# dhansmair/flamingo-mini

Measured on AMD Instinct MI355X. Metric: images/sec (fwd+bwd) flamingo-mini bs=32, higher is better.
Workload: dtype bf16

## Files before the change

### flamingo-mini_amd/csrc/ff_api.hip

```cpp
#include <stdarg.h>
#include <stdio.h>
#include <math.h>
#include <stdlib.h>
#include "ff_common.h"
#include "ff_internal.h"

namespace ff {

static thread_local char g_err[512] = "";
void set_error(const char* fmt, ...) {
    va_list ap;
    va_start(ap, fmt);
    vsnprintf(g_err, sizeof(g_err), fmt, ap);
    va_end(ap);
}
#ifdef FF_DEBUG
int dbg_switch(const char* name, int dflt) {
    const char* e = getenv(name);
    return e ? atoi(e) : dflt;
}
#endif
int check_launch(const char* what) {
    hipError_t e = hipGetLastError();
    if (e != hipSuccess) {
// ... 76 lines not shown
    }
    o.x_last = a.take(rows_q * s.D * s.es);
    o.mean_o = a.take<float>(rows_q * 4);
    o.rstd_o = a.take<float>(rows_q * 4);
    return align_up(a.used);
}

static size_t rs_ws_bytes(const RsDims& s) {
    size_t w = 0;
    auto g = [&](int M, int N, int K, int nz) { w = std::max(w, gemm_workspace_bytes(s.dt, M, N, K, nz, 0)); };
    g(s.Mq, s.inner, s.D, 1); g(s.Mkv, s.inner, s.D, 2); g(s.Mq, s.D, s.inner, 1); g(s.Mq, s.ffi, s.D, 1); g(s.Mq, s.D, s.ffi, 1);
    for (int nz = 1; nz <= 4; nz++) {
        g(s.D, s.ffi, s.Mq, nz); g(s.ffi, s.D, s.Mq, nz); g(s.D, s.inner, s.Mq, nz); g(s.inner, s.D, s.Mq, nz); g(s.inner, s.D, s.Mkv, nz);
    }
    g(s.Mkv, s.D, s.inner, 1);
    w = std::max(w, layernorm_bwd_workspace(s.Mf, s.D));
    w = std::max(w, layernorm_bwd_workspace(s.Mq, s.D));
    w = std::max(w, rows_reduce_workspace(s.Mq, s.D, s.q, 1));
    w = std::max(w, rows_reduce_workspace(s.Mf, s.D, s.F, s.v));
    return align_up(w) + align_up(s.attn_ws);
}
struct RsChain {
    void *ws, *dxn, *dO, *dkv, *dln;
    size_t ws_bytes, gws;
    float* attn_ws;
};
struct RsLayerGrads {
    void *dx_mid, *dH, *dQs, *dK, *dV;
};
static void rs_take_ws(const RsDims& s, Arena& a, RsChain& c) {
// ... 98 lines not shown
    if (partial)
        return layernorm_bwd(a, dy, x, add, gamma, mean, rstd, dx, dx_res, dg, db, partial, layernorm_bwd_partial_bytes(a.rows, a.cols), st, nullptr, pending);
    return layernorm_bwd(a, dy, x, add, gamma, mean, rstd, dx, dx_res, dg, db, W.ws, W.gws, st);
}

static int rs_layer_backward(const RsDims& s, const void* const* p, void* const* g, const void* x_f, const void* tpe, const float* mean_m,
                             const float* rstd_m, const void* x_in, RowMap x_map, const RsLayerSaved& L, const void* dx_out, void* dx_in,
                             void* dx_f, const void* dx_f_res, const RsChain& W, const RsLayerGrads& T, float* const* lnp, LnPending* ln_sets,
                             hipStream_t st) {
    const RowMap pD = s.pD, pI = s.pI, pF = s.pF;
    FF_TRY(Gemm(s.dt, s.Mq, s.ffi, s.D).a(0, pD).b(1, pF).c(pF).act_bwd(s.act).problem(dx_out, p[11], T.dH, nullptr, L.Hpre).run(W.ws, W.gws, st));
    FF_TRY(Gemm(s.dt, s.Mq, s.D, s.ffi).a(0, pF).b(1, pD).c(pD).problem(T.dH, p[10], W.dxn).run(W.ws, W.gws, st));
    FF_TRY(rs_ln_bwd(W, lnp[0], &ln_sets[0], s.ln_latents(), W.dxn, L.x_mid, nullptr, p[8], L.mean_f, L.rstd_f, T.dx_mid, dx_out, g[8], g[9], st));
    FF_TRY(Gemm(s.dt, s.Mq, s.inner, s.D).a(0, pD).b(1, pI).c(pI).problem(T.dx_mid, p[7], W.dO).run(W.ws, W.gws, st));
    FF_TRY(attention_bwd(rs_attn_desc(s), L.Qs, L.K, L.V, nullptr, L.O, W.dO, L.lse, T.dQs, T.dK, T.dV, W.attn_ws, s.attn_ws, st));
    FF_TRY(Gemm(s.dt, s.Mkv, s.D, s.inner).a(0, pI).b(1, pD).c(pD).problem(T.dK, p[5], W.dkv).run(W.ws, W.gws, st));
    FF_TRY(Gemm(s.dt, s.Mkv, s.D, s.inner).a(0, pI).b(1, pD).c(pD).problem(T.dV, p[6], W.dkv, nullptr, nullptr, W.dkv).run(W.ws, W.gws, st));
    FF_TRY(Gemm(s.dt, s.Mq, s.D, s.inner).a(0, pI).b(1, pD).c(pD).res_map(s.kv_lat).scale(s.scale)
               .problem(T.dQs, p[4], W.dln, nullptr, nullptr, s.kv_latent_rows(W.dkv)).run(W.ws, W.gws, st));
    FF_TRY(rs_ln_bwd(W, lnp[1], &ln_sets[1], ln_args(s.dt, s.Mq, s.D, x_map, pD, pD), W.dln, x_in, nullptr, p[2], L.mean_l, L.rstd_l, dx_in, T.dx_mid, g[2],
                     g[3], st));
    return rs_ln_bwd(W, lnp[2], &ln_sets[2], s.ln_media(s.kv_media), W.dkv, x_f, tpe, p[0], mean_m, rstd_m, dx_f, dx_f_res, g[0], g[1], st);
}

static int rs_input_grads(const RsDims& s, const void* dx0, const void* dxf, void* d_latents, void* d_tpe, void* ws, size_t ws_bytes, hipStream_t st) {
    FF_TRY(rows_reduce(s.dt, s.Mq, s.D, s.pD, s.q, 1, dx0, d_latents, ws, ws_bytes, st));
    if (s.nte > s.T) FF_TRY(zero_bytes((char*)d_tpe + (size_t)s.T * s.D * s.es, (size_t)(s.nte - s.T) * s.D * s.es, st));
    return rows_reduce(s.dt, s.Mf, s.D, s.pD, s.F, s.v, dxf, d_tpe, ws, ws_bytes, st);
}

static int resampler_fwd(const ff_resampler_desc* d, const void* x_f, const void* const* P, void* out, void* saved, size_t saved_bytes,
                         void* scratch, size_t scratch_bytes, hipStream_t st) {
// ... 517 lines not shown
    }
    if (finish_ln) FF_TRY(layernorm_bwd_finish(s.dt, ln_sets, 2 * n, st));
    FF_TRY(g3.run(ws, ws_bytes, st));
    FF_TRY(g1.run(ws, ws_bytes, st));
    FF_TRY(go.run(ws, ws_bytes, st));
    return gq.run(ws, ws_bytes, st);
}

static int kvp_check(const ff_kvproj_desc* d) {
    FF_CHECK(d, FF_ERR_SHAPE, "kv_project: null descriptor");
    FF_CHECK(d->dtype == FF_DTYPE_F32 || d->dtype == FF_DTYPE_BF16, FF_ERR_UNSUPPORTED, "kv_project: dtype %d", d->dtype);
    FF_CHECK(d->n_layers > 0 && d->rows > 0 && d->dim_visual > 0 && d->kv_dim > 0 && (long long)d->rows * d->dim_visual < (1LL << 31), FF_ERR_SHAPE,
             "kv_project: bad dimensions");
    return FF_OK;
}
static size_t kvp_gemm_ws(const ff_kvproj_desc* d) {
    size_t w = 0;
    for (int z = 1; z <= kKvProjGroup; z++)
        w = std::max({w, gemm_workspace_bytes(d->dtype, d->rows, d->kv_dim, d->dim_visual, z, 0),
                      gemm_workspace_bytes(d->dtype, d->kv_dim, d->dim_visual, d->rows, z, 0),
                      gemm_workspace_bytes(d->dtype, d->rows, d->dim_visual, d->kv_dim, z, 0)});
    return align_up(w);
}
static size_t kvp_ws_bytes(const ff_kvproj_desc* d, bool with_dvf) {
    const size_t es = d->dtype == FF_DTYPE_BF16 ? 2 : 4;
    size_t w = kvp_gemm_ws(d);
    if (with_dvf)
        w += align_up((size_t)d->n_layers * d->rows * d->dim_visual * es) +
             align_up(rows_reduce_workspace(d->n_layers, d->rows * d->dim_visual, d->n_layers, d->n_layers));
    return w;
}
static int kv_project_fwd(const ff_kvproj_desc* d, const void* vf, const void* const* w_kv, void* const* kv_out, void* ws, size_t ws_bytes,
                          hipStream_t st) {
    FF_TRY(kvp_check(d));
    FF_CHECK(vf && w_kv && kv_out && ws && ws_bytes >= kvp_gemm_ws(d), FF_ERR_WORKSPACE, "kv_project_fwd: null argument or workspace too small");
    const RowMap pV = plain_rows(d->dim_visual), pKV = plain_rows(d->kv_dim);
    for (int l0 = 0; l0 < d->n_layers; l0 += kKvProjGroup) {
        Gemm g(d->dtype, d->rows, d->kv_dim, d->dim_visual);
        g.a(0, pV).b(0, pV).c(pKV);
        for (int l = l0; l < std::min(d->n_layers, l0 + kKvProjGroup); l++) g.problem(vf, w_kv[l], kv_out[l]);
        FF_TRY(g.run(ws, ws_bytes, st));
    }
    return FF_OK;
}
static int kv_project_bwd(const ff_kvproj_desc* d, const void* vf, const void* const* w_kv, const void* const* dkv, void* const* dw_kv,
                          void* dvf, void* ws, size_t ws_bytes, hipStream_t st) {
    FF_TRY(kvp_check(d));
    FF_CHECK(vf && w_kv && dkv && dw_kv && ws && ws_bytes >= kvp_ws_bytes(d, dvf != nullptr), FF_ERR_WORKSPACE,
             "kv_project_bwd: null argument or workspace too small");
    const size_t es = d->dtype == FF_DTYPE_BF16 ? 2 : 4, gws = kvp_gemm_ws(d);
    const RowMap pV = plain_rows(d->dim_visual), pKV = plain_rows(d->kv_dim);
    char* terms = (char*)ws + gws;
    const size_t term_bytes = (size_t)d->rows * d->dim_visual * es;
    for (int l0 = 0; l0 < d->n_layers; l0 += kKvProjGroup) {
        const int l1 = std::min(d->n_layers, l0 + kKvProjGroup);
        Gemm gw(d->dtype, d->kv_dim, d->dim_visual, d->rows);
        gw.a(1, pKV).b(1, pV).c(pV);
        for (int l = l0; l < l1; l++) gw.problem(dkv[l], vf, dw_kv[l]);
        FF_TRY(gw.run(ws, gws, st));
        if (dvf) {
            Gemm gx(d->dtype, d->rows, d->dim_visual, d->kv_dim);
            gx.a(0, pKV).b(1, pV).c(pV);
            for (int l = l0; l < l1; l++) gx.problem(dkv[l], w_kv[l], terms + (size_t)l * term_bytes);
            FF_TRY(gx.run(ws, gws, st));
        }
    }
    if (dvf) {
        const int cols = d->rows * d->dim_visual;
        FF_TRY(rows_reduce(d->dtype, d->n_layers, cols, plain_rows(cols), d->n_layers, d->n_layers, terms, dvf,
                           terms + align_up((size_t)d->n_layers * term_bytes), rows_reduce_workspace(d->n_layers, cols, d->n_layers, d->n_layers), st));
    }
    return FF_OK;
}

}

extern "C" int ff_version(void) { return 6; }
extern "C" const char* ff_arch(void) { return "gfx950"; }
extern "C" const char* ff_last_error(void) { return ff::g_err; }

extern "C" size_t ff_resampler_saved_bytes(const ff_resampler_desc* d) {
    if (ff::rs_check(d) != FF_OK) return 0;
    ff::RsSaved S;
    return ff::rs_saved_layout(ff::RsDims(*d), nullptr, 0, S);
}
// ... 146 lines not shown
```

### flamingo-mini_amd/csrc/ff_gemm.hip

```cpp
#include <atomic>
#include <type_traits>
#include "ff_common.h"
#include <stdlib.h>
#include "ff_internal.h"
#include "ff_gemm_tiles.h"

namespace ff {

template <typename T>
FF_DEV void epilogue4(const GemmParams& P, const GemmProblem& pr, int m, int n, float (&v)[4]) {
    typedef __attribute__((ext_vector_type(4))) T vec4;
    const long long off = P.c_map.off(m) + n;
    const bool full = (n + 3 < P.N);
#pragma unroll
    for (int r = 0; r < 4; r++) v[r] *= P.scale;
    auto load4 = [&](const void* base, long long at, float (&o)[4]) {
        const T* p = (const T*)base + at;
        if (full) {
            vec4 t = *(const vec4*)p;
#pragma unroll
            for (int r = 0; r < 4; r++) o[r] = to_f32(t[r]);
        } else {
#pragma unroll
            for (int r = 0; r < 4; r++) o[r] = (n + r < P.N) ? to_f32(p[r]) : 0.f;
// ... 328 lines not shown
        } else dma_tile_fast<BN, BL, NW>(r, st, v, soff, w);
    }
    static FF_DEV void slow(__amdgpu_buffer_rsrc_t r, bf16* st, const RowMap& map, int n_base, int n_lim, int k0, int k_end, int w, int l, bf16* dummy = nullptr) {
        if constexpr (SPLIT) {
            dma_tile<128, BL, NW>(r, st, map, n_base, n_lim, k0, k_end, w, l);
            if (NW == 8 && w >= 4) dma_tile<32, BL, 4>(r, dummy, map, n_base + 128, 0, k0, k_end, 0, l);
            else dma_tile<32, BL, 4>(r, st + 128 * kBK, map, n_base + 128, n_lim, k0, k_end, w & 3, l);
        } else dma_tile<BN, BL, NW>(r, st, map, n_base, n_lim, k0, k_end, w, l);
    }
    static FF_DEV bf16x8 frag(const bf16* s, int col0, int ks) {
        if constexpr (SPLIT && BL == 1) return col0 < 128 ? frag_read2<128, 1>(s, col0, ks) : frag_read2<32, 1>(s + 128 * kBK, col0 - 128, ks);
        else return frag_read2<BN, BL>(s, col0, ks);
    }
};

template <int BM, int BN, int AL, int BL, int NS, int WPC, int NPW = 4, int NCW = 4>
__global__ __launch_bounds__((NCW + NPW) * 64, WPC * (NCW + NPW) / 4) void gemm_bf16_pc_kernel(const void* hA, const void* hB, int hM, int hN, int hK, int h_split, int h_kps,
                                                           int h_nz, int h_xcd, int h_ald, int h_bld, int h_seg, const GemmParams P) {
    extern __shared__ __attribute__((aligned(16))) unsigned char smem_raw[];
    bf16* smem = (bf16*)smem_raw;
    constexpr int A_ELEMS = BM * kBK, B_ELEMS = BN * kBK, STAGE = A_ELEMS + B_ELEMS;
    constexpr int CM = NCW / 2;
    constexpr int WM = BM / CM, WN = BN / 2, MT = WM / 16, NT = WN / 16;
    static_assert((NCW == 4 || NCW == 8) && WM % 16 == 0, "consumer layout");
    typedef BStage<BN, BL, NPW> BS;
    constexpr int PER_TILE = BM / (NPW * 8) + BS::PER_WAVE;
    static_assert(WN % 16 == 0 && BM % 32 == 0 && BN % 32 == 0, "tile shape");
    static_assert((AL == 0 || BM == 256 || BM == 128 || BM == 64) && (BL == 0 || BN == 128 || BN == 64 || BN == 160), "M-major staging exists for 64 / 128 / 256-wide A tiles and 64 / 128 / 160-wide B tiles only");
    static_assert(PER_TILE * (NS - 1) <= 63, "vmcnt overflow");

    RowMap a_map{h_ald, 0, 0}, b_map{h_bld, 0, 0};
    if (h_seg) { a_map = P.a_map; b_map = P.b_map; }
    const void* opA = hA;
    const void* opB = hB;
    const int tiles_m = (hM + BM - 1) / BM, tiles_n = (hN + BN - 1) / BN;
    const TileCoord tc = tile_coord(h_nz, h_split, h_xcd & 255, h_xcd >> 8, tiles_m, tiles_n);
    if (tc.z > 0) { opA = P.p[tc.z].A; opB = P.p[tc.z].B; }
    const int m_base = tc.tm * BM, n_base = tc.tn * BN;
    const int k_begin = tc.split * h_kps;
    const int k_end = min(hK, k_begin + h_kps);
    const int t = threadIdx.x, l = t & 63;
    const int w = __builtin_amdgcn_readfirstlane(t >> 6);
    const bool producer = w >= NCW;
    const int pw = producer ? w - NCW : w;
    const int wm = (w & (NCW - 1)) >> 1, wn = w & 1;
    bf16* dummy = smem + NS * STAGE + (pw & 3) * 512;
    const __amdgpu_buffer_rsrc_t ra = __builtin_amdgcn_make_buffer_rsrc((void*)opA, 0, 0x7fffffff, 0x00020000);
    const __amdgpu_buffer_rsrc_t rb = __builtin_amdgcn_make_buffer_rsrc((void*)opB, 0, 0x7fffffff, 0x00020000);
    const int nk = (k_end - k_begin + kBK - 1) / kBK;

    f32x4 acc[MT][NT];
#pragma unroll
    for (int i = 0; i < MT; i++)
#pragma unroll
        for (int j = 0; j < NT; j++) acc[i][j] = f32x4{0.f, 0.f, 0.f, 0.f};

    unsigned va[BM / (NPW * 8)], vb[BS::PER_WAVE];
    const bool a_plain = AL == 0 || a_map.rows_per_seg <= 0, b_plain = BL == 0 || b_map.rows_per_seg <= 0;
    const unsigned a_step = AL == 0 ? 2u : (unsigned)a_map.ld * 2u, b_step = BL == 0 ? 2u : (unsigned)b_map.ld * 2u;
    auto issue = [&](int tile) {
        bf16* st = smem + (tile % NS) * STAGE;
        const int k0 = k_begin + tile * kBK;
        const bool full = k0 + kBK <= k_end;
        if (full && a_plain) dma_tile_fast<BM, AL, NPW>(ra, st, va, (unsigned)k0 * a_step, pw);
        else dma_tile<BM, AL, NPW>(ra, st, a_map, m_base, hM, k0, k_end, pw, l);
        if (full && b_plain) BS::fast(rb, st + A_ELEMS, vb, (unsigned)k0 * b_step, pw, dummy);
        else BS::slow(rb, st + A_ELEMS, b_map, n_base, hN, k0, k_end, pw, l, dummy);
    };
    if (producer) {
        dma_prepare<BM, AL, NPW>(a_map, m_base, hM, pw, l, va);
        BS::prepare(b_map, n_base, hN, pw, l, vb);
#pragma unroll
        for (int s = 0; s < NS - 1; s++)
            if (s < nk) issue(s);
    }
    FF_GEMM_ARGS(Q, pr, P);
    if (tc.z > 0) pr = P.p[tc.z];
#ifdef FF_GEMM_PCMODE
    constexpr int pcmode = FF_GEMM_PCMODE;
#else
    constexpr int pcmode = 0;
#endif
    if (producer) {
        for (int kt = 0; kt < nk; kt++) {
            if (pcmode == 2) { __builtin_amdgcn_s_barrier(); continue; }
            const int younger = min(nk - 1 - kt, NS - 2);
            if (NS >= 4 && younger == 2) wait_vmcnt<2 * PER_TILE>();
            else if (NS >= 3 && younger >= 1) wait_vmcnt<PER_TILE>();
            else wait_vmcnt<0>();
            __builtin_amdgcn_s_barrier();
            if (kt + NS - 1 < nk) issue(kt + NS - 1);
        }
// ... 317 lines not shown
#pragma unroll
        for (int j = 0; j < 4; j++) s[(k + j) * kFLd + row] = reg[j];
    } else {
        const int k = t >> 4, row = (t & 15) * 4;
        *(f32x4*)(s + k * kFLd + row) = f32x4{reg[0], reg[1], reg[2], reg[3]};
    }
}

template <int AL, int BL> __global__ __launch_bounds__(256) void gemm_f32_kernel(const GemmParams P) {
    __shared__ __attribute__((aligned(16))) float sA[kFBK * kFLd];
    __shared__ __attribute__((aligned(16))) float sB[kFBK * kFLd];
    const int tiles_m = (P.M + kFBM - 1) / kFBM, tiles_n = (P.N + kFBM - 1) / kFBM;
    const TileCoord tc = tile_coord(P.nz, P.split_k, P.xcd_ms, P.xcd_ns, tiles_m, tiles_n);
    const GemmProblem& pr = P.p[tc.z];
    const int m_base = tc.tm * kFBM, n_base = tc.tn * kFBM;
    const int k_begin = tc.split * P.k_per_split;
    const int k_end = min(P.K, k_begin + P.k_per_split);
    const float* A = (const float*)pr.A;
    const float* B = (const float*)pr.B;
    const int t = threadIdx.x, w = t >> 6, l = t & 63, c = l & 15, g = l >> 4;
    const int wm = w >> 1, wn = w & 1;
    const bool a_vec = P.a_vec_ok, b_vec = P.b_vec_ok;

    f32x4 acc[2][2];
#pragma unroll
    for (int i = 0; i < 2; i++)
#pragma unroll
        for (int j = 0; j < 2; j++) acc[i][j] = f32x4{0.f, 0.f, 0.f, 0.f};

    for (int k0 = k_begin; k0 < k_end; k0 += kFBK) {
        float ra[4], rb[4];
        f32_tile_load<AL>(A, P.a_map, m_base, P.M, k0, k_end, a_vec, ra);
        f32_tile_load<BL>(B, P.b_map, n_base, P.N, k0, k_end, b_vec, rb);
        __syncthreads();
        f32_tile_store<AL>(sA, ra);
        f32_tile_store<BL>(sB, rb);
        __syncthreads();
#pragma unroll
        for (int ks = 0; ks < kFBK / 4; ks++) {
            float fa[2], fb[2];
#pragma unroll
            for (int i = 0; i < 2; i++) fa[i] = sA[(ks * 4 + g) * kFLd + wm * 32 + i * 16 + c];
#pragma unroll
            for (int j = 0; j < 2; j++) fb[j] = sB[(ks * 4 + g) * kFLd + wn * 32 + j * 16 + c];
#pragma unroll
// ... 92 lines not shown
}
int profile_begin(int dtype, int tile, int a_layout, int b_layout, int M, int N, int K, int nz, int split_k, hipStream_t st) {
    if (!g_prof.on.load(std::memory_order_relaxed)) return -1;
    const int i = g_prof.n.fetch_add(1);
    if (i >= g_prof.cap) return -1;
    ff_gemm_profile_record& r = g_prof.rec[i];
    r.dtype = dtype; r.tile = tile; r.a_layout = a_layout; r.b_layout = b_layout;
    r.M = M; r.N = N; r.K = K; r.nz = nz; r.split_k = split_k; r.ms = 0.f;
    hipEventRecord(g_prof.ev[2 * i], st);
    return i;
}
void profile_end(int i, hipStream_t st) {
    if (i >= 0) hipEventRecord(g_prof.ev[2 * i + 1], st);
}
static int prof_begin(const GemmParams& P, int dtype, int bm, hipStream_t st) {
    return profile_begin(dtype, bm, P.a_layout, P.b_layout, P.M, P.N, P.K, P.nz, P.split_k, st);
}
static void prof_end(int i, hipStream_t st) { profile_end(i, st); }

static int env_int(const char* name, int dflt) { return dbg_switch(name, dflt); }

struct TilePlan { int tile, split; };
static TilePlan plan_bf16(int M, int N, int K, int nz, int want_split, int a_layout = 0, int b_layout = 0, int ft = 0) {
    const long long t128 = (long long)cdiv(M, 128) * cdiv(N, 128) * nz, t64 = (long long)cdiv(M, 64) * cdiv(N, 64) * nz;
    TilePlan p;
    static const int env_tile = env_int("FF_GEMM_TILE", 0);
    if (ft == 0) ft = env_tile;
    static const int pc_bl1 = env_int("FF_GEMM_PC_BL1", 1);
    const bool pc_ok = a_layout == 0 && (b_layout == 0 || (pc_bl1 && N % 8 == 0));
    const bool skinny_ok = a_layout == 0 && b_layout == 0;
    const bool rows_ok = skinny_ok && M <= 32 && nz == 1 && K % 32 == 0;
// ... 43 lines not shown
    } else if (t64 >= 200) p = TilePlan{64, 1};
    else {
        int s = (int)std::min<long long>(4, cdiv(256, t64));
        while (s > 1 && K / (64 * s) < 4) s--;
        p = TilePlan{64, s};
    }
    if (want_split > 0) p.split = want_split;
    static const int pc128 = env_int("FF_GEMM_PC128", 2);
    if (pc128 && p.tile == 128) p.tile = 128002;
    if (pc128 >= 2 && p.tile == 6412) p.tile = 128002;
    static const int pc64 = env_int("FF_GEMM_PC64", 1);
    if (pc64 && p.tile == 64) p.tile = 64002;
    return p;
}

template <int BM, int BN, int AL, int BL, int NS> static int launch_bf16_dma(const GemmParams& P, hipStream_t st) {
    constexpr size_t lds = (size_t)NS * (BM + BN) * kBK * sizeof(bf16);
    if (lds > 64 * 1024) {
        static bool attr_done[64] = {};
        int dev = 0;
        (void)hipGetDevice(&dev);
        if (dev < 0 || dev >= 64 || !attr_done[dev]) {
            hipError_t e = hipFuncSetAttribute((const void*)gemm_bf16_dma_kernel<BM, BN, AL, BL, NS>,
                                               hipFuncAttributeMaxDynamicSharedMemorySize, (int)lds);
            FF_CHECK(e == hipSuccess, FF_ERR_LAUNCH, "hipFuncSetAttribute(gemm dma lds=%zu): %s", lds, hipGetErrorString(e));
            if (dev >= 0 && dev < 64) attr_done[dev] = true;
        }
    }
    const int grid = cdiv(P.M, BM) * cdiv(P.N, BN) * P.split_k * P.nz;
    const int seg = P.a_map.rows_per_seg > 0 || P.b_map.rows_per_seg > 0 || P.a_map.ld >= (1LL << 31) || P.b_map.ld >= (1LL << 31);
    gemm_bf16_dma_kernel<BM, BN, AL, BL, NS><<<dim3(grid), dim3(256), lds, st>>>(P.p[0].A, P.p[0].B, P.M, P.N, P.K, P.split_k, P.k_per_split, P.nz,
                                                                           P.xcd_ms | (P.xcd_ns << 8), (int)P.a_map.ld, (int)P.b_map.ld, seg, P);
    return check_launch("gemm_bf16_dma");
}
template <int BM, int BN, int NS> static int dispatch_bf16_dma(const GemmParams& P, hipStream_t st) {
    if (P.a_layout == 0 && P.b_layout == 0) return launch_bf16_dma<BM, BN, 0, 0, NS>(P, st);
    if (P.a_layout == 0 && P.b_layout == 1) return launch_bf16_dma<BM, BN, 0, 1, NS>(P, st);
    if (P.a_layout == 1 && P.b_layout == 0) return launch_bf16_dma<BM, BN, 1, 0, NS>(P, st);
    return launch_bf16_dma<BM, BN, 1, 1, NS>(P, st);
}
template <int BM, int BN> static int run_bf16_dma_tile(const GemmParams& P, int ns, hipStream_t st) {
    return ns == 2 ? dispatch_bf16_dma<BM, BN, 2>(P, st) : ns == 4 ? dispatch_bf16_dma<BM, BN, 4>(P, st) : dispatch_bf16_dma<BM, BN, 3>(P, st);
}
template <int BM, int BN, int AL, int BL, int NS, int WPC, int NPW = 4, int NCW = 4> static int launch_bf16_pc(const GemmParams& P, hipStream_t st) {
    constexpr size_t lds = (size_t)NS * (BM + BN) * kBK * sizeof(bf16) + (NPW == 8 && BN == 160 ? 4096 : 0);
    static bool attr_done[64] = {};
    int dev = 0;
    (void)hipGetDevice(&dev);
    if (dev < 0 || dev >= 64 || !attr_done[dev]) {
        hipError_t e = hipFuncSetAttribute((const void*)gemm_bf16_pc_kernel<BM, BN, AL, BL, NS, WPC, NPW, NCW>, hipFuncAttributeMaxDynamicSharedMemorySize, (int)lds);
        FF_CHECK(e == hipSuccess, FF_ERR_LAUNCH, "hipFuncSetAttribute(gemm pc lds=%zu): %s", lds, hipGetErrorString(e));
        if (dev >= 0 && dev < 64) attr_done[dev] = true;
    }
    const int grid = cdiv(P.M, BM) * cdiv(P.N, BN) * P.split_k * P.nz;
    const int seg = P.a_map.rows_per_seg > 0 || P.b_map.rows_per_seg > 0 || P.a_map.ld >= (1LL << 31) || P.b_map.ld >= (1LL << 31);
    gemm_bf16_pc_kernel<BM, BN, AL, BL, NS, WPC, NPW, NCW><<<dim3(grid), dim3((NCW + NPW) * 64), lds, st>>>(P.p[0].A, P.p[0].B, P.M, P.N, P.K, P.split_k, P.k_per_split,
                                                                                 P.nz, P.xcd_ms | (P.xcd_ns << 8), (int)P.a_map.ld,
                                                                                 (int)P.b_map.ld, seg, P);
    return check_launch("gemm_bf16_pc");
}
template <int NS> static int dispatch_bf16_pc128(const GemmParams& P, hipStream_t st) {
    if (P.a_layout == 0 && P.b_layout == 0) return launch_bf16_pc<128, 128, 0, 0, NS, 2>(P, st);
    if (P.a_layout == 0 && P.b_layout == 1) return launch_bf16_pc<128, 128, 0, 1, NS, 2>(P, st);
    if (P.a_layout == 1 && P.b_layout == 0) return launch_bf16_pc<128, 128, 1, 0, NS, 2>(P, st);
    return launch_bf16_pc<128, 128, 1, 1, NS, 2>(P, st);
}
static int run_bf16_dma(const GemmParams& P, hipStream_t st) {
    static const int ns_env = env_int("FF_GEMM_STAGES", 0);
    const int ns = P.force_stages > 0 ? P.force_stages : ns_env > 0 ? ns_env : 2;
    if (P.tile == 128160) {
        static const int npw_full = env_int("FF_GEMM_NPW", 8), npw_split = env_int("FF_GEMM_NPW_SPLIT", 4);
        const int npw = P.split_k > 1 ? npw_split : npw_full;
        const int pns = P.force_stages > 0 ? P.force_stages : ns_env > 0 ? ns_env : npw == 8 ? 4 : 3;
        static const int ncw_env = env_int("FF_GEMM_NCW", 4), ncw_split_env = env_int("FF_GEMM_NCW_SPLIT", 4);
        const int ncw = P.force_tile == 128168 ? 8 : (P.split_k > 1 ? ncw_split_env : ncw_env);
        if (ncw == 8) {
            if (P.b_layout == 0) return pns == 3 ? launch_bf16_pc<128, 160, 0, 0, 3, 1, 4, 8>(P, st) : launch_bf16_pc<128, 160, 0, 0, 4, 1, 4, 8>(P, st);
            return pns == 3 ? launch_bf16_pc<128, 160, 0, 1, 3, 1, 4, 8>(P, st) : launch_bf16_pc<128, 160, 0, 1, 4, 1, 4, 8>(P, st);
        }
        if (npw == 8) {
            if (P.b_layout == 0) return pns == 4 ? launch_bf16_pc<128, 160, 0, 0, 4, 1, 8>(P, st) : launch_bf16_pc<128, 160, 0, 0, 3, 1, 8>(P, st);
            return pns == 4 ? launch_bf16_pc<128, 160, 0, 1, 4, 1, 8>(P, st) : launch_bf16_pc<128, 160, 0, 1, 3, 1, 8>(P, st);
        }
        if (P.b_layout == 0) return pns == 4 ? launch_bf16_pc<128, 160, 0, 0, 4, 1>(P, st) : launch_bf16_pc<128, 160, 0, 0, 3, 1>(P, st);
// ... 29 lines not shown
    int s = (int)(256 / tiles);
    s = std::min(s, K / 512);
    s = std::min(s, 16);
    return std::max(s, 1);
}

size_t gemm_workspace_bytes(int dtype, int M, int N, int K, int nz, int split_k) {
    if (split_k <= 0) split_k = gemm_pick_split(dtype, M, N, K, nz);
    return split_k > 1 ? (size_t)split_k * nz * M * N * sizeof(float) : 0;
}

int gemm_launch(GemmParams P, int dtype, void* workspace, size_t ws_bytes, hipStream_t st, int* leave_partial) {
    if (leave_partial) *leave_partial = 1;
    FF_CHECK(P.M > 0 && P.N > 0 && P.K > 0 && P.nz >= 1 && P.nz <= kGemmMaxZ, FF_ERR_SHAPE, "gemm: bad shape M=%d N=%d K=%d nz=%d",
             P.M, P.N, P.K, P.nz);
    P.tile = kFBM;
    if (dtype == FF_DTYPE_BF16) {
        const TilePlan plan = plan_bf16(P.M, P.N, P.K, P.nz, P.split_k, P.a_layout, P.b_layout, P.force_tile);
        P.tile = plan.tile;
        P.split_k = plan.split;
    } else if (P.split_k <= 0) P.split_k = gemm_pick_split(dtype, P.M, P.N, P.K, P.nz);
    const int kq = dtype == FF_DTYPE_BF16 ? kBK : kFBK;
    P.k_per_split = cdiv(cdiv(P.K, P.split_k), kq) * kq;
    P.split_k = cdiv(P.K, P.k_per_split);
    P.partial = nullptr;
    if (P.split_k > 1) {
        const size_t need = gemm_workspace_bytes(dtype, P.M, P.N, P.K, P.nz, P.split_k);
        FF_CHECK(workspace && ws_bytes >= need, FF_ERR_WORKSPACE, "gemm split-K workspace: need %zu have %zu", need, ws_bytes);
        FF_CHECK(P.N % 4 == 0, FF_ERR_UNSUPPORTED, "gemm split-K needs N %% 4 == 0 (N=%d)", P.N);
        P.partial = (float*)workspace;
    }
    {
        const int tm_edge = dtype == FF_DTYPE_BF16 ? (P.tile == 256128 || P.tile == 256256 ? 256 : P.tile == 128 || P.tile == 128160 || P.tile == 128002 ? 128 : P.tile == 3264 || P.tile == 3216 ? 32 : 64) : kFBM;
        const int tn_edge = dtype == FF_DTYPE_BF16 ? (P.tile == 3216 ? 16 : P.tile == 64 || P.tile == 64002 || P.tile == 3264 ? 64 : P.tile == 128160 ? 160 : P.tile == 256256 ? 256 : 128) : kFBM;
        const int tiles_m = cdiv(P.M, tm_edge), tiles_n = cdiv(P.N, tn_edge);
        double best = 1e300;
        P.xcd_ms = 1; P.xcd_ns = 1;
        for (int ms = 1; ms <= 8; ms *= 2) {
            const int ns = 8 / ms;
            if (ms > tiles_m || ns > tiles_n) continue;
            const double cost = (double)P.M / ms + (double)P.N / ns;
            if (cost < best) { best = cost; P.xcd_ms = ms; P.xcd_ns = ns; }
        }
        static const int disable = env_int("FF_GEMM_XCD2D", 1) == 0;
        if (disable) { P.xcd_ms = 1; P.xcd_ns = 1; }
    }
    const int vec = dtype == FF_DTYPE_BF16 ? 8 : 4;
    auto map_ok = [&](const RowMap& m) { return m.ld % vec == 0 && (m.rows_per_seg <= 0 || m.seg_stride % vec == 0); };
    const int a_contig = P.a_layout == 0 ? P.K : P.M, b_contig = P.b_layout == 0 ? P.K : P.N;
    P.a_vec_ok = map_ok(P.a_map) && a_contig % vec == 0;
    P.b_vec_ok = map_ok(P.b_map) && b_contig % vec == 0;
    for (int z = 0; z < P.nz; z++) {
        P.a_vec_ok = P.a_vec_ok && ((uintptr_t)P.p[z].A % 16 == 0);
        P.b_vec_ok = P.b_vec_ok && ((uintptr_t)P.p[z].B % 16 == 0);
    }
    P.c_vec8 = P.N % vec == 0 && map_ok(P.c_map) && map_ok(P.r_map);
    for (int z = 0; z < P.nz; z++)
        P.c_vec8 = P.c_vec8 && ((uintptr_t)P.p[z].C | (uintptr_t)P.p[z].aux_out | (uintptr_t)P.p[z].aux_in | (uintptr_t)P.p[z].residual) % 16 == 0;
    int rc;
    const int prof_id = prof_begin(P, dtype, P.tile, st);
    if (dtype == FF_DTYPE_BF16) {
        FF_CHECK(P.a_vec_ok && P.b_vec_ok, FF_ERR_UNSUPPORTED,
                 "bf16 gemm needs 16-byte aligned operands with contiguous dims %% 8 == 0 (M=%d N=%d K=%d)", P.M, P.N, P.K);
        FF_CHECK(P.N % 4 == 0 && P.c_map.ld % 4 == 0, FF_ERR_UNSUPPORTED, "bf16 gemm needs N %% 4 == 0 (N=%d)", P.N);
        auto span_ok = [&](const RowMap& m, int rows, int contig) {
            const long long last = (m.rows_per_seg > 0 ? (long long)((rows - 1) / m.rows_per_seg) * m.seg_stride + (long long)((rows - 1) % m.rows_per_seg) * m.ld
                                                      : (long long)(rows - 1) * m.ld) + contig;
            return last < (1LL << 30);
        };
// ... 9 lines not shown
        !P.p[0].residual) {
        *leave_partial = P.split_k;
        return FF_OK;
    }
    if (P.split_k > 1) {
        const long long total = (long long)P.nz * P.M * ((P.N + 7) / 8);
        FF_CHECK(total < (1LL << 31), FF_ERR_UNSUPPORTED, "gemm split-K output too large (M=%d N=%d nz=%d)", P.M, P.N, P.nz);
        const int grid = (int)((total + 255) / 256);
        if (dtype == FF_DTYPE_BF16) hipLaunchKernelGGL(gemm_splitk_epilogue_kernel<bf16>, dim3(grid), dim3(256), 0, st, P);
        else hipLaunchKernelGGL(gemm_splitk_epilogue_kernel<float>, dim3(grid), dim3(256), 0, st, P);
        FF_TRY(check_launch("gemm_splitk_epilogue"));
    }
    return FF_OK;
}

}

#ifdef FF_GEMM_TIMELINE
extern "C" int ff_debug_timeline_read(unsigned long long* out, int n_blocks) {
    return (int)hipMemcpyFromSymbol(out, HIP_SYMBOL(ff::g_timeline), sizeof(unsigned long long) * 8 * n_blocks);
}
#endif

extern "C" size_t ff_gemm_workspace_bytes(const ff_gemm_desc* d) {
    int split = d->split_k;
    if (split <= 0 && d->tile > 0 && d->dtype == FF_DTYPE_BF16) split = ff::plan_bf16(d->M, d->N, d->K, 1, 0, d->a_layout, d->b_layout, d->tile).split;
    return ff::gemm_workspace_bytes(d->dtype, d->M, d->N, d->K, 1, split);
}

extern "C" int ff_gemm(const ff_gemm_desc* d, const void* A, const void* B, void* C, void* aux_out, const void* aux_in,
// ... 64 lines not shown
```

### flamingo-mini_amd/csrc/ff_internal.h

```cpp
#pragma once
#include <algorithm>
#include "ff_common.h"

namespace ff {

constexpr int kGemmMaxZ = 12;
constexpr int kKvProjGroup = 4;
struct GemmProblem {
    const void* A;
    const void* B;
    void* C;
    void* aux_out;
    const void* aux_in;
    const void* residual;
    const void* gate;
};
struct GemmParams {
    int M, N, K;
    int a_layout, b_layout;
    RowMap a_map, b_map, c_map, r_map;
    float scale;
    int act, act_bwd;
    int split_k, k_per_split;
    int tile;
    int force_tile, force_stages;
    int xcd_ms, xcd_ns;
    float* partial;
    int a_vec_ok, b_vec_ok;
    int c_vec8;
    int nz;
    GemmProblem p[kGemmMaxZ];
};
int gemm_pick_split(int dtype, int M, int N, int K, int nz);
size_t gemm_workspace_bytes(int dtype, int M, int N, int K, int nz, int split_k);
int gemm_launch(GemmParams P, int dtype, void* workspace, size_t ws_bytes, hipStream_t st, int* leave_partial = nullptr);

struct Gemm {
    GemmParams P;
    int dtype;
    Gemm(int dtype_, int M, int N, int K) : dtype(dtype_) {
        P = GemmParams{};
        P.M = M; P.N = N; P.K = K;
        P.scale = 1.f; P.act = FF_ACT_NONE; P.act_bwd = FF_ACT_NONE; P.split_k = 0; P.nz = 0;
        P.a_map = plain_rows(K); P.b_map = plain_rows(K); P.c_map = plain_rows(N); P.r_map = P.c_map;
    }
    Gemm& a(int layout, RowMap m) { P.a_layout = layout; P.a_map = m; return *this; }
    Gemm& b(int layout, RowMap m) { P.b_layout = layout; P.b_map = m; return *this; }
    Gemm& c(RowMap m) { P.c_map = m; P.r_map = m; return *this; }
    Gemm& res_map(RowMap m) { P.r_map = m; return *this; }
    Gemm& scale(float s) { P.scale = s; return *this; }
    Gemm& act(int a) { P.act = a; return *this; }
    Gemm& act_bwd(int a) { P.act_bwd = a; return *this; }
    Gemm& problem(const void* A, const void* B, void* C, void* aux_out = nullptr, const void* aux_in = nullptr,
                  const void* residual = nullptr, const void* gate = nullptr) {
        P.p[P.nz++] = GemmProblem{A, B, C, aux_out, aux_in, residual, gate};
        return *this;
    }
    size_t workspace() const { return gemm_workspace_bytes(dtype, P.M, P.N, P.K, std::max(P.nz, 1), P.split_k); }
    int run(void* ws, size_t ws_bytes, hipStream_t st, int* leave_partial = nullptr) const { return gemm_launch(P, dtype, ws, ws_bytes, st, leave_partial); }
};

int profile_begin(int dtype, int tile, int a_layout, int b_layout, int M, int N, int K, int nz, int split_k, hipStream_t st);
void profile_end(int i, hipStream_t st);

struct LnArgs {
    int dtype;
    int rows, cols;
    RowMap x_map, y_map, dx_map;
    int add_rows_per_seg, add_div;
    float eps;
    int stats_given;
    int dy_splits = 0;
    long long dy_slab = 0;
};
// ... 94 lines not shown
```

Before: 781.1.

## Add K-segment list GEMMs to fuse summed backward products and drop reduction buffers

```diff
diff --git a/flamingo-mini_amd/csrc/ff_api.hip b/flamingo-mini_amd/csrc/ff_api.hip
--- a/flamingo-mini_amd/csrc/ff_api.hip
+++ b/flamingo-mini_amd/csrc/ff_api.hip
@@ -114,6 +114,7 @@
         g(s.D, s.ffi, s.Mq, nz); g(s.ffi, s.D, s.Mq, nz); g(s.D, s.inner, s.Mq, nz); g(s.inner, s.D, s.Mq, nz); g(s.inner, s.D, s.Mkv, nz);
     }
     g(s.Mkv, s.D, s.inner, 1);
+    w = std::max(w, gemm_segments_workspace_bytes(s.dt, s.Mkv, s.D, s.inner, 2));
     w = std::max(w, layernorm_bwd_workspace(s.Mf, s.D));
     w = std::max(w, layernorm_bwd_workspace(s.Mq, s.D));
     w = std::max(w, rows_reduce_workspace(s.Mq, s.D, s.q, 1));
@@ -242,8 +243,7 @@
     FF_TRY(rs_ln_bwd(W, lnp[0], &ln_sets[0], s.ln_latents(), W.dxn, L.x_mid, nullptr, p[8], L.mean_f, L.rstd_f, T.dx_mid, dx_out, g[8], g[9], st));
     FF_TRY(Gemm(s.dt, s.Mq, s.inner, s.D).a(0, pD).b(1, pI).c(pI).problem(T.dx_mid, p[7], W.dO).run(W.ws, W.gws, st));
     FF_TRY(attention_bwd(rs_attn_desc(s), L.Qs, L.K, L.V, nullptr, L.O, W.dO, L.lse, T.dQs, T.dK, T.dV, W.attn_ws, s.attn_ws, st));
-    FF_TRY(Gemm(s.dt, s.Mkv, s.D, s.inner).a(0, pI).b(1, pD).c(pD).problem(T.dK, p[5], W.dkv).run(W.ws, W.gws, st));
-    FF_TRY(Gemm(s.dt, s.Mkv, s.D, s.inner).a(0, pI).b(1, pD).c(pD).problem(T.dV, p[6], W.dkv, nullptr, nullptr, W.dkv).run(W.ws, W.gws, st));
+    FF_TRY(Gemm(s.dt, s.Mkv, s.D, s.inner).a(0, pI).b(1, pD).c(pD).problem(T.dK, p[5], W.dkv).segment(T.dV, p[6]).run(W.ws, W.gws, st));
     FF_TRY(Gemm(s.dt, s.Mq, s.D, s.inner).a(0, pI).b(1, pD).c(pD).res_map(s.kv_lat).scale(s.scale)
                .problem(T.dQs, p[4], W.dln, nullptr, nullptr, s.kv_latent_rows(W.dkv)).run(W.ws, W.gws, st));
     FF_TRY(rs_ln_bwd(W, lnp[1], &ln_sets[1], ln_args(s.dt, s.Mq, s.D, x_map, pD, pD), W.dln, x_in, nullptr, p[2], L.mean_l, L.rstd_l, dx_in, T.dx_mid, g[2],
@@ -791,20 +791,25 @@
              "kv_project: bad dimensions");
     return FF_OK;
 }
+static int kvp_wgrad_split(const ff_kvproj_desc* d, int nz) {
+    if (d->dtype != FF_DTYPE_BF16) return 0;
+    const long long t128 = (long long)cdiv(d->kv_dim, 128) * cdiv(d->dim_visual, 128) * nz;
+    if (t128 < 128 || t128 > 256) return 0;
+    int s = (int)(512 / t128);
+    while (s > 1 && d->rows / (64 * s) < 8) s--;
+    return s > 1 ? s : 0;
+}
 static size_t kvp_gemm_ws(const ff_kvproj_desc* d) {
     size_t w = 0;
     for (int z = 1; z <= kKvProjGroup; z++)
-        w = std::max({w, gemm_workspace_bytes(d->dtype, d->rows, d->kv_dim, d->dim_visual, z, 0),
-                      gemm_workspace_bytes(d->dtype, d->kv_dim, d->dim_visual, d->rows, z, 0),
-                      gemm_workspace_bytes(d->dtype, d->rows, d->dim_visual, d->kv_dim, z, 0)});
+        w = std::max(w, gemm_workspace_bytes(d->dtype, d->rows, d->kv_dim, d->dim_visual, z, 0));
+    for (int z = 1; z <= kKvWgradGroup; z++)
+        w = std::max(w, gemm_workspace_bytes(d->dtype, d->kv_dim, d->dim_visual, d->rows, z, kvp_wgrad_split(d, z)));
     return align_up(w);
 }
 static size_t kvp_ws_bytes(const ff_kvproj_desc* d, bool with_dvf) {
-    const size_t es = d->dtype == FF_DTYPE_BF16 ? 2 : 4;
     size_t w = kvp_gemm_ws(d);
-    if (with_dvf)
-        w += align_up((size_t)d->n_layers * d->rows * d->dim_visual * es) +
-             align_up(rows_reduce_workspace(d->n_layers, d->rows * d->dim_visual, d->n_layers, d->n_layers));
+    if (with_dvf) w = std::max(w, align_up(gemm_segments_workspace_bytes(d->dtype, d->rows, d->dim_visual, d->kv_dim, d->n_layers)));
     return w;
 }
 static int kv_project_fwd(const ff_kvproj_desc* d, const void* vf, const void* const* w_kv, void* const* kv_out, void* ws, size_t ws_bytes,
@@ -825,27 +830,20 @@
     FF_TRY(kvp_check(d));
     FF_CHECK(vf && w_kv && dkv && dw_kv && ws && ws_bytes >= kvp_ws_bytes(d, dvf != nullptr), FF_ERR_WORKSPACE,
              "kv_project_bwd: null argument or workspace too small");
-    const size_t es = d->dtype == FF_DTYPE_BF16 ? 2 : 4, gws = kvp_gemm_ws(d);
     const RowMap pV = plain_rows(d->dim_visual), pKV = plain_rows(d->kv_dim);
-    char* terms = (char*)ws + gws;
-    const size_t term_bytes = (size_t)d->rows * d->dim_visual * es;
-    for (int l0 = 0; l0 < d->n_layers; l0 += kKvProjGroup) {
-        const int l1 = std::min(d->n_layers, l0 + kKvProjGroup);
+    for (int l0 = 0; l0 < d->n_layers; l0 += kKvWgradGroup) {
+        const int l1 = std::min(d->n_layers, l0 + kKvWgradGroup);
         Gemm gw(d->dtype, d->kv_dim, d->dim_visual, d->rows);
         gw.a(1, pKV).b(1, pV).c(pV);
+        gw.P.split_k = kvp_wgrad_split(d, l1 - l0);
         for (int l = l0; l < l1; l++) gw.problem(dkv[l], vf, dw_kv[l]);
-        FF_TRY(gw.run(ws, gws, st));
-        if (dvf) {
-            Gemm gx(d->dtype, d->rows, d->dim_visual, d->kv_dim);
-            gx.a(0, pKV).b(1, pV).c(pV);
-            for (int l = l0; l < l1; l++) gx.problem(dkv[l], w_kv[l], terms + (size_t)l * term_bytes);
-            FF_TRY(gx.run(ws, gws, st));
-        }
+        FF_TRY(gw.run(ws, ws_bytes, st));
     }
     if (dvf) {
-        const int cols = d->rows * d->dim_visual;
-        FF_TRY(rows_reduce(d->dtype, d->n_layers, cols, plain_rows(cols), d->n_layers, d->n_layers, terms, dvf,
-                           terms + align_up((size_t)d->n_layers * term_bytes), rows_reduce_workspace(d->n_layers, cols, d->n_layers, d->n_layers), st));
+        Gemm gx(d->dtype, d->rows, d->dim_visual, d->kv_dim);
+        gx.a(0, pKV).b(1, pV).c(pV).problem(dkv[0], w_kv[0], dvf);
+        for (int l = 1; l < d->n_layers; l++) gx.segment(dkv[l], w_kv[l]);
+        FF_TRY(gx.run(ws, ws_bytes, st));
     }
     return FF_OK;
 }
diff --git a/flamingo-mini_amd/csrc/ff_gemm.hip b/flamingo-mini_amd/csrc/ff_gemm.hip
--- a/flamingo-mini_amd/csrc/ff_gemm.hip
+++ b/flamingo-mini_amd/csrc/ff_gemm.hip
@@ -366,7 +366,7 @@
     }
 };
 
-template <int BM, int BN, int AL, int BL, int NS, int WPC, int NPW = 4, int NCW = 4>
+template <int BM, int BN, int AL, int BL, int NS, int WPC, int NPW = 4, int NCW = 4, int KS = 0>
 __global__ __launch_bounds__((NCW + NPW) * 64, WPC * (NCW + NPW) / 4) void gemm_bf16_pc_kernel(const void* hA, const void* hB, int hM, int hN, int hK, int h_split, int h_kps,
                                                            int h_nz, int h_xcd, int h_ald, int h_bld, int h_seg, const GemmParams P) {
     extern __shared__ __attribute__((aligned(16))) unsigned char smem_raw[];
@@ -386,20 +386,26 @@
     const void* opA = hA;
     const void* opB = hB;
     const int tiles_m = (hM + BM - 1) / BM, tiles_n = (hN + BN - 1) / BN;
-    const TileCoord tc = tile_coord(h_nz, h_split, h_xcd & 255, h_xcd >> 8, tiles_m, tiles_n);
-    if (tc.z > 0) { opA = P.p[tc.z].A; opB = P.p[tc.z].B; }
+    const TileCoord tc = tile_coord(KS ? 1 : h_nz, h_split, h_xcd & 255, h_xcd >> 8, tiles_m, tiles_n);
+    if (!KS && tc.z > 0) { opA = P.p[tc.z].A; opB = P.p[tc.z].B; }
     const int m_base = tc.tm * BM, n_base = tc.tn * BN;
-    const int k_begin = tc.split * h_kps;
-    const int k_end = min(hK, k_begin + h_kps);
+    const int k_begin = KS ? 0 : tc.split * h_kps;
+    const int k_end = KS ? hK : min(hK, k_begin + h_kps);
+    int ks_seg = KS ? tc.split * h_kps : 0, ks_k0 = 0;
+    const int ks_end = KS ? min(h_nz, ks_seg + h_kps) : 1;
+    if (KS && ks_seg > 0) { opA = P.seg[ks_seg].A; opB = P.seg[ks_seg].B; }
     const int t = threadIdx.x, l = t & 63;
     const int w = __builtin_amdgcn_readfirstlane(t >> 6);
     const bool producer = w >= NCW;
     const int pw = producer ? w - NCW : w;
     const int wm = (w & (NCW - 1)) >> 1, wn = w & 1;
     bf16* dummy = smem + NS * STAGE + (pw & 3) * 512;
-    const __amdgpu_buffer_rsrc_t ra = __builtin_amdgcn_make_buffer_rsrc((void*)opA, 0, 0x7fffffff, 0x00020000);
-    const __amdgpu_buffer_rsrc_t rb = __builtin_amdgcn_make_buffer_rsrc((void*)opB, 0, 0x7fffffff, 0x00020000);
-    const int nk = (k_end - k_begin + kBK - 1) / kBK;
+    __amdgpu_buffer_rsrc_t ra = __builtin_amdgcn_make_buffer_rsrc((void*)opA, 0, 0x7fffffff, 0x00020000);
+    __amdgpu_buffer_rsrc_t rb = __builtin_amdgcn_make_buffer_rsrc((void*)opB, 0, 0x7fffffff, 0x00020000);
+    const int nk = (KS ? max(ks_end - ks_seg, 0) : 1) * ((k_end - k_begin + kBK - 1) / kBK);
+    const void* nxA = nullptr;
+    const void* nxB = nullptr;
+    if (KS && producer && ks_seg + 1 < ks_end) { nxA = P.seg[ks_seg + 1].A; nxB = P.seg[ks_seg + 1].B; }
 
     f32x4 acc[MT][NT];
 #pragma unroll
@@ -412,12 +418,22 @@
     const unsigned a_step = AL == 0 ? 2u : (unsigned)a_map.ld * 2u, b_step = BL == 0 ? 2u : (unsigned)b_map.ld * 2u;
     auto issue = [&](int tile) {
         bf16* st = smem + (tile % NS) * STAGE;
-        const int k0 = k_begin + tile * kBK;
+        const int k0 = KS ? ks_k0 : k_begin + tile * kBK;
         const bool full = k0 + kBK <= k_end;
         if (full && a_plain) dma_tile_fast<BM, AL, NPW>(ra, st, va, (unsigned)k0 * a_step, pw);
         else dma_tile<BM, AL, NPW>(ra, st, a_map, m_base, hM, k0, k_end, pw, l);
         if (full && b_plain) BS::fast(rb, st + A_ELEMS, vb, (unsigned)k0 * b_step, pw, dummy);
         else BS::slow(rb, st + A_ELEMS, b_map, n_base, hN, k0, k_end, pw, l, dummy);
+        if constexpr (KS != 0) {
+            ks_k0 += kBK;
+            if (ks_k0 >= k_end) {
+                ks_k0 = 0;
+                ks_seg++;
+                ra = __builtin_amdgcn_make_buffer_rsrc((void*)nxA, 0, 0x7fffffff, 0x00020000);
+                rb = __builtin_amdgcn_make_buffer_rsrc((void*)nxB, 0, 0x7fffffff, 0x00020000);
+                if (ks_seg + 1 < ks_end) { nxA = P.seg[ks_seg + 1].A; nxB = P.seg[ks_seg + 1].B; }
+            }
+        }
     };
     if (producer) {
         dma_prepare<BM, AL, NPW>(a_map, m_base, hM, pw, l, va);
@@ -427,7 +443,7 @@
             if (s < nk) issue(s);
     }
     FF_GEMM_ARGS(Q, pr, P);
-    if (tc.z > 0) pr = P.p[tc.z];
+    if (!KS && tc.z > 0) pr = P.p[tc.z];
 #ifdef FF_GEMM_PCMODE
     constexpr int pcmode = FF_GEMM_PCMODE;
 #else
@@ -775,8 +791,10 @@
     const TileCoord tc = tile_coord(P.nz, P.split_k, P.xcd_ms, P.xcd_ns, tiles_m, tiles_n);
     const GemmProblem& pr = P.p[tc.z];
     const int m_base = tc.tm * kFBM, n_base = tc.tn * kFBM;
-    const int k_begin = tc.split * P.k_per_split;
-    const int k_end = min(P.K, k_begin + P.k_per_split);
+    const bool ks = P.nseg > 1;
+    const int seg_begin = ks ? tc.split * P.seg_per_split : 0, seg_end = ks ? min(P.nseg, seg_begin + P.seg_per_split) : 1;
+    const int k_begin = ks ? 0 : tc.split * P.k_per_split;
+    const int k_end = ks ? P.K : min(P.K, k_begin + P.k_per_split);
     const float* A = (const float*)pr.A;
     const float* B = (const float*)pr.B;
     const int t = threadIdx.x, w = t >> 6, l = t & 63, c = l & 15, g = l >> 4;
@@ -789,7 +807,9 @@
 #pragma unroll
         for (int j = 0; j < 2; j++) acc[i][j] = f32x4{0.f, 0.f, 0.f, 0.f};
 
+    for (int sg = seg_begin; sg < seg_end; sg++)
     for (int k0 = k_begin; k0 < k_end; k0 += kFBK) {
+        if (ks) { A = (const float*)P.seg[sg].A; B = (const float*)P.seg[sg].B; }
         float ra[4], rb[4];
         f32_tile_load<AL>(A, P.a_map, m_base, P.M, k0, k_end, a_vec, ra);
         f32_tile_load<BL>(B, P.b_map, n_base, P.N, k0, k_end, b_vec, rb);
@@ -912,7 +932,7 @@
     if (i >= 0) hipEventRecord(g_prof.ev[2 * i + 1], st);
 }
 static int prof_begin(const GemmParams& P, int dtype, int bm, hipStream_t st) {
-    return profile_begin(dtype, bm, P.a_layout, P.b_layout, P.M, P.N, P.K, P.nz, P.split_k, st);
+    return profile_begin(dtype, bm, P.a_layout, P.b_layout, P.M, P.N, P.nseg > 1 ? P.K * P.nseg : P.K, P.nz, P.split_k, st);
 }
 static void prof_end(int i, hipStream_t st) { profile_end(i, st); }
 
@@ -986,6 +1006,34 @@
     return p;
 }
 
+static TilePlan plan_kseg(int dtype, int M, int N, int K_seg, int nseg, int want_split) {
+    const long long Kt = (long long)K_seg * nseg;
+    TilePlan p;
+    if (dtype != FF_DTYPE_BF16) {
+        const long long tiles = (long long)cdiv(M, kFBM) * cdiv(N, kFBM);
+        p.tile = kFBM;
+        p.split = (tiles >= 128 || Kt < 1024) ? 1 : (int)std::max<long long>(1, std::min<long long>(std::min<long long>(256 / tiles, Kt / 512), 16));
+    } else {
+        const long long t128 = (long long)cdiv(M, 128) * cdiv(N, 128), t64 = (long long)cdiv(M, 64) * cdiv(N, 64);
+        if (t128 >= 200) p = TilePlan{128002, 1};
+        else if (Kt >= 2048) {
+            int s = (int)std::min<long long>(8, std::max<long long>(1, 512 / t128));
+            while (s > 1 && Kt / (64 * s) < 8) s--;
+            p = TilePlan{128002, s};
+        } else if (t64 >= 200) p = TilePlan{64002, 1};
+        else {
+            int s = (int)std::min<long long>(4, cdiv(256, t64));
+            while (s > 1 && Kt / (64 * s) < 4) s--;
+            p = TilePlan{64002, s};
+        }
+    }
+    if (want_split > 0) p.split = want_split;
+    p.split = std::max(1, std::min(p.split, nseg));
+    const int per = cdiv(nseg, p.split);
+    p.split = cdiv(nseg, per);
+    return p;
+}
+
 template <int BM, int BN, int AL, int BL, int NS> static int launch_bf16_dma(const GemmParams& P, hipStream_t st) {
     constexpr size_t lds = (size_t)NS * (BM + BN) * kBK * sizeof(bf16);
     if (lds > 64 * 1024) {
@@ -1014,22 +1062,28 @@
 template <int BM, int BN> static int run_bf16_dma_tile(const GemmParams& P, int ns, hipStream_t st) {
     return ns == 2 ? dispatch_bf16_dma<BM, BN, 2>(P, st) : ns == 4 ? dispatch_bf16_dma<BM, BN, 4>(P, st) : dispatch_bf16_dma<BM, BN, 3>(P, st);
 }
-template <int BM, int BN, int AL, int BL, int NS, int WPC, int NPW = 4, int NCW = 4> static int launch_bf16_pc(const GemmParams& P, hipStream_t st) {
+template <int BM, int BN, int AL, int BL, int NS, int WPC, int NPW = 4, int NCW = 4, int KS = 0> static int launch_bf16_pc(const GemmParams& P, hipStream_t st) {
     constexpr size_t lds = (size_t)NS * (BM + BN) * kBK * sizeof(bf16) + (NPW == 8 && BN == 160 ? 4096 : 0);
     static bool attr_done[64] = {};
     int dev = 0;
     (void)hipGetDevice(&dev);
     if (dev < 0 || dev >= 64 || !attr_done[dev]) {
-        hipError_t e = hipFuncSetAttribute((const void*)gemm_bf16_pc_kernel<BM, BN, AL, BL, NS, WPC, NPW, NCW>, hipFuncAttributeMaxDynamicSharedMemorySize, (int)lds);
+        hipError_t e = hipFuncSetAttribute((const void*)gemm_bf16_pc_kernel<BM, BN, AL, BL, NS, WPC, NPW, NCW, KS>, hipFuncAttributeMaxDynamicSharedMemorySize, (int)lds);
         FF_CHECK(e == hipSuccess, FF_ERR_LAUNCH, "hipFuncSetAttribute(gemm pc lds=%zu): %s", lds, hipGetErrorString(e));
         if (dev >= 0 && dev < 64) attr_done[dev] = true;
     }
     const int grid = cdiv(P.M, BM) * cdiv(P.N, BN) * P.split_k * P.nz;
     const int seg = P.a_map.rows_per_seg > 0 || P.b_map.rows_per_seg > 0 || P.a_map.ld >= (1LL << 31) || P.b_map.ld >= (1LL << 31);
-    gemm_bf16_pc_kernel<BM, BN, AL, BL, NS, WPC, NPW, NCW><<<dim3(grid), dim3((NCW + NPW) * 64), lds, st>>>(P.p[0].A, P.p[0].B, P.M, P.N, P.K, P.split_k, P.k_per_split,
-                                                                                 P.nz, P.xcd_ms | (P.xcd_ns << 8), (int)P.a_map.ld,
-                                                                                 (int)P.b_map.ld, seg, P);
+    gemm_bf16_pc_kernel<BM, BN, AL, BL, NS, WPC, NPW, NCW, KS><<<dim3(grid), dim3((NCW + NPW) * 64), lds, st>>>(P.p[0].A, P.p[0].B, P.M, P.N, P.K, P.split_k,
+                                                                                 KS ? P.seg_per_split : P.k_per_split, KS ? P.nseg : P.nz,
+                                                                                 P.xcd_ms | (P.xcd_ns << 8), (int)P.a_map.ld, (int)P.b_map.ld, seg, P);
     return check_launch("gemm_bf16_pc");
+}
+template <int BM, int BN, int NS> static int dispatch_bf16_pc_kseg(const GemmParams& P, hipStream_t st) {
+    if (P.a_layout == 0 && P.b_layout == 0) return launch_bf16_pc<BM, BN, 0, 0, NS, 2, 4, 4, 1>(P, st);
+    if (P.a_layout == 0 && P.b_layout == 1) return launch_bf16_pc<BM, BN, 0, 1, NS, 2, 4, 4, 1>(P, st);
+    if (P.a_layout == 1 && P.b_layout == 0) return launch_bf16_pc<BM, BN, 1, 0, NS, 2, 4, 4, 1>(P, st);
+    return launch_bf16_pc<BM, BN, 1, 1, NS, 2, 4, 4, 1>(P, st);
 }
 template <int NS> static int dispatch_bf16_pc128(const GemmParams& P, hipStream_t st) {
     if (P.a_layout == 0 && P.b_layout == 0) return launch_bf16_pc<128, 128, 0, 0, NS, 2>(P, st);
@@ -1040,6 +1094,11 @@
 static int run_bf16_dma(const GemmParams& P, hipStream_t st) {
     static const int ns_env = env_int("FF_GEMM_STAGES", 0);
     const int ns = P.force_stages > 0 ? P.force_stages : ns_env > 0 ? ns_env : 2;
+    if (P.nseg > 1) {
+        if (P.tile == 128002) return dispatch_bf16_pc_kseg<128, 128, 2>(P, st);
+        if (P.tile == 64002) return dispatch_bf16_pc_kseg<64, 64, 3>(P, st);
+        FF_CHECK(false, FF_ERR_UNSUPPORTED, "gemm: tile %d does not implement K-segment lists (128002 and 64002 do)", P.tile);
+    }
     if (P.tile == 128160) {
         static const int npw_full = env_int("FF_GEMM_NPW", 8), npw_split = env_int("FF_GEMM_NPW_SPLIT", 4);
         const int npw = P.split_k > 1 ? npw_split : npw_full;
@@ -1099,15 +1158,34 @@
     if (leave_partial) *leave_partial = 1;
     FF_CHECK(P.M > 0 && P.N > 0 && P.K > 0 && P.nz >= 1 && P.nz <= kGemmMaxZ, FF_ERR_SHAPE, "gemm: bad shape M=%d N=%d K=%d nz=%d",
              P.M, P.N, P.K, P.nz);
+    const bool kseg = P.nseg != 0;
+    if (kseg) {
+        FF_CHECK(P.nseg >= 2 && P.nseg <= kGemmMaxSeg && P.nz == 1, FF_ERR_SHAPE, "gemm: a K-segment list has 2..%d segments and one problem (nseg=%d nz=%d)",
+                 kGemmMaxSeg, P.nseg, P.nz);
+        for (int i = 0; i < P.nseg; i++) FF_CHECK(P.seg[i].A && P.seg[i].B, FF_ERR_SHAPE, "gemm: null operand in K-segment %d", i);
+        FF_CHECK(dtype != FF_DTYPE_BF16 || P.force_tile == 0 || P.force_tile == 128002 || P.force_tile == 64002, FF_ERR_UNSUPPORTED,
+                 "gemm: tile %d does not implement K-segment lists (128002 and 64002 do)", P.force_tile);
+        P.p[0].A = P.seg[0].A; P.p[0].B = P.seg[0].B;
+    }
     P.tile = kFBM;
-    if (dtype == FF_DTYPE_BF16) {
+    if (kseg) {
+        TilePlan plan = plan_kseg(dtype, P.M, P.N, P.K, P.nseg, P.split_k);
+        if (dtype == FF_DTYPE_BF16 && P.force_tile) plan.tile = P.force_tile;
+        P.tile = plan.tile;
+        P.split_k = plan.split;
+    } else if (dtype == FF_DTYPE_BF16) {
         const TilePlan plan = plan_bf16(P.M, P.N, P.K, P.nz, P.split_k, P.a_layout, P.b_layout, P.force_tile);
         P.tile = plan.tile;
         P.split_k = plan.split;
     } else if (P.split_k <= 0) P.split_k = gemm_pick_split(dtype, P.M, P.N, P.K, P.nz);
     const int kq = dtype == FF_DTYPE_BF16 ? kBK : kFBK;
-    P.k_per_split = cdiv(cdiv(P.K, P.split_k), kq) * kq;
-    P.split_k = cdiv(P.K, P.k_per_split);
+    if (kseg) {
+        P.seg_per_split = cdiv(P.nseg, P.split_k);
+        P.k_per_split = P.seg_per_split * P.K;
+    } else {
+        P.k_per_split = cdiv(cdiv(P.K, P.split_k), kq) * kq;
+        P.split_k = cdiv(P.K, P.k_per_split);
+    }
     P.partial = nullptr;
     if (P.split_k > 1) {
         const size_t need = gemm_workspace_bytes(dtype, P.M, P.N, P.K, P.nz, P.split_k);
@@ -1138,6 +1216,10 @@
     for (int z = 0; z < P.nz; z++) {
         P.a_vec_ok = P.a_vec_ok && ((uintptr_t)P.p[z].A % 16 == 0);
         P.b_vec_ok = P.b_vec_ok && ((uintptr_t)P.p[z].B % 16 == 0);
+    }
+    for (int i = 0; i < P.nseg; i++) {
+        P.a_vec_ok = P.a_vec_ok && ((uintptr_t)P.seg[i].A % 16 == 0);
+        P.b_vec_ok = P.b_vec_ok && ((uintptr_t)P.seg[i].B % 16 == 0);
     }
     P.c_vec8 = P.N % vec == 0 && map_ok(P.c_map) && map_ok(P.r_map);
     for (int z = 0; z < P.nz; z++)
@@ -1177,6 +1259,35 @@
     return FF_OK;
 }
 
+size_t gemm_segments_workspace_bytes(int dtype, int M, int N, int K_seg, int n) {
+    size_t w = 0;
+    for (int s0 = 0; s0 < n; s0 += kGemmMaxSeg) {
+        const int c = std::min(n - s0, kGemmMaxSeg);
+        const int split = c > 1 ? plan_kseg(dtype, M, N, K_seg, c, 0).split : gemm_pick_split(dtype, M, N, K_seg, 1);
+        w = std::max(w, gemm_workspace_bytes(dtype, M, N, K_seg, 1, split));
+    }
+    return w;
+}
+
+int gemm_launch_segments(GemmParams P, const GemmSeg* segs, int n, int dtype, void* workspace, size_t ws_bytes, hipStream_t st) {
+    FF_CHECK(segs && n >= 1 && P.nz == 1, FF_ERR_SHAPE, "gemm: a K-segment list needs one problem and at least one segment (n=%d nz=%d)", n, P.nz);
+    FF_CHECK(n <= kGemmMaxSeg || (P.act < 0 && P.act_bwd < 0 && !P.p[0].aux_out && !P.p[0].gate), FF_ERR_UNSUPPORTED,
+             "gemm: more than %d K-segments need a scale / residual-only epilogue (n=%d)", kGemmMaxSeg, n);
+    for (int s0 = 0; s0 < n; s0 += kGemmMaxSeg) {
+        const int c = std::min(n - s0, kGemmMaxSeg);
+        GemmParams Q = P;
+        if (s0 > 0) { Q.p[0].residual = P.p[0].C; Q.r_map = P.c_map; }
+        Q.nseg = 0;
+        Q.p[0].A = segs[s0].A; Q.p[0].B = segs[s0].B;
+        if (c > 1) {
+            Q.nseg = c;
+            for (int i = 0; i < c; i++) Q.seg[i] = segs[s0 + i];
+        }
+        FF_TRY(gemm_launch(Q, dtype, workspace, ws_bytes, st));
+    }
+    return FF_OK;
+}
+
 }
 
 #ifdef FF_GEMM_TIMELINE
diff --git a/flamingo-mini_amd/csrc/ff_internal.h b/flamingo-mini_amd/csrc/ff_internal.h
--- a/flamingo-mini_amd/csrc/ff_internal.h
+++ b/flamingo-mini_amd/csrc/ff_internal.h
@@ -1,11 +1,18 @@
 #pragma once
 #include <algorithm>
+#include <vector>
 #include "ff_common.h"
 
 namespace ff {
 
 constexpr int kGemmMaxZ = 12;
 constexpr int kKvProjGroup = 4;
+constexpr int kKvWgradGroup = 8;
+constexpr int kGemmMaxSeg = 48;
+struct GemmSeg {
+    const void* A;
+    const void* B;
+};
 struct GemmProblem {
     const void* A;
     const void* B;
@@ -30,14 +37,19 @@
     int c_vec8;
     int nz;
     GemmProblem p[kGemmMaxZ];
+    int nseg, seg_per_split;
+    GemmSeg seg[kGemmMaxSeg];
 };
 int gemm_pick_split(int dtype, int M, int N, int K, int nz);
 size_t gemm_workspace_bytes(int dtype, int M, int N, int K, int nz, int split_k);
 int gemm_launch(GemmParams P, int dtype, void* workspace, size_t ws_bytes, hipStream_t st, int* leave_partial = nullptr);
+int gemm_launch_segments(GemmParams P, const GemmSeg* segs, int n, int dtype, void* workspace, size_t ws_bytes, hipStream_t st);
+size_t gemm_segments_workspace_bytes(int dtype, int M, int N, int K_seg, int n);
 
 struct Gemm {
     GemmParams P;
     int dtype;
+    std::vector<GemmSeg> segs;
     Gemm(int dtype_, int M, int N, int K) : dtype(dtype_) {
         P = GemmParams{};
         P.M = M; P.N = N; P.K = K;
@@ -56,8 +68,19 @@
         P.p[P.nz++] = GemmProblem{A, B, C, aux_out, aux_in, residual, gate};
         return *this;
     }
-    size_t workspace() const { return gemm_workspace_bytes(dtype, P.M, P.N, P.K, std::max(P.nz, 1), P.split_k); }
-    int run(void* ws, size_t ws_bytes, hipStream_t st, int* leave_partial = nullptr) const { return gemm_launch(P, dtype, ws, ws_bytes, st, leave_partial); }
+    Gemm& segment(const void* A, const void* B) {
+        if (segs.empty()) segs.push_back(GemmSeg{P.p[0].A, P.p[0].B});
+        segs.push_back(GemmSeg{A, B});
+        return *this;
+    }
+    size_t workspace() const {
+        if (!segs.empty()) return gemm_segments_workspace_bytes(dtype, P.M, P.N, P.K, (int)segs.size());
+        return gemm_workspace_bytes(dtype, P.M, P.N, P.K, std::max(P.nz, 1), P.split_k);
+    }
+    int run(void* ws, size_t ws_bytes, hipStream_t st, int* leave_partial = nullptr) const {
+        if (!segs.empty()) return gemm_launch_segments(P, segs.data(), (int)segs.size(), dtype, ws, ws_bytes, st);
+        return gemm_launch(P, dtype, ws, ws_bytes, st, leave_partial);
+    }
 };
 
 int profile_begin(int dtype, int tile, int a_layout, int b_layout, int M, int N, int K, int nz, int split_k, hipStream_t st);
```

Result: no change. 785.1 (median of 6 runs) (+0.5%).
